# martende/findex

Measured on AMD Instinct MI355X. Metric: rank_queries_per_sec, higher is better.
Workload: dtype u64

## Files before the change

findex_amd/csrc/fmx_host.h:

```cpp
#pragma once
#include <hip/hip_runtime.h>
#include <stdint.h>

#include <atomic>
#include <memory>
#include <mutex>
#include <string>
#include <vector>

#include "fmx_device.h"
#include "fmx_hostpar.h"

namespace fmx {

struct CallCtx {
  static constexpr int kBufs = 8;
  hipStream_t stream = nullptr;
  hipEvent_t ev_a = nullptr, ev_b = nullptr;
  void *buf[kBufs] = {nullptr};
  size_t cap[kBufs] = {0};
  std::vector<hipEvent_t> chunk_ev;
  void *pin = nullptr;
  size_t pin_cap = 0;
  size_t total() const { size_t t = 0; for (size_t c : cap) t += c; return t; }
};

struct KTab {
  const uint4 *tab = nullptr;
  const uint4 *level[16] = {nullptr};
  const uint4 *const *level_dev = nullptr;
  const uint8_t *dense = nullptr;
  uint32_t k = 0, sigma = 0;
  const unsigned long long *row1 = nullptr;
  const uint4 *ext = nullptr, *ovf = nullptr;
  uint32_t ext_k = 0;
};

struct HostRank {
  std::vector<uint8_t> blob;
  size_t stride = 0;
};

struct TablePolicy {
  std::atomic<int> ktab{1};
  std::atomic<int> ktab_ext{-1};
  std::atomic<int> jump_mode{7};
  std::atomic<int> jump_pairs{-1};
  std::atomic<int> search_lanes{-1};
  std::atomic<int> jump_chars{9};
  std::atomic<long long> tables_after{-1};
  std::atomic<uint64_t> budget_bytes{~0ull};
  std::atomic<uint32_t> budget_ppb{0};
  std::atomic<int> locate_sample{32};
  TablePolicy() = default;
  TablePolicy(const TablePolicy &o) { *this = o; }
  TablePolicy &operator=(const TablePolicy &o) {
    ktab.store(o.ktab.load()); ktab_ext.store(o.ktab_ext.load()); jump_mode.store(o.jump_mode.load()); jump_pairs.store(o.jump_pairs.load());
    search_lanes.store(o.search_lanes.load());
    jump_chars.store(o.jump_chars.load()); tables_after.store(o.tables_after.load());
    budget_bytes.store(o.budget_bytes.load()); budget_ppb.store(o.budget_ppb.load());
    locate_sample.store(o.locate_sample.load());
    return *this;
  }
};
TablePolicy &default_policy();
int policy_set(TablePolicy &p, const char *key, const char *value, const char **why);

struct Index {
  uint64_t serial = 0;
  int device = 0;
  int cu_count = 256;
  uint64_t n = 0, eof = 0, nblocks = 0;
  uint32_t nslots = 0;
  int64_t counts[256] = {0};
  uint64_t cf[256] = {0};
  uint16_t slot[256] = {0};
  bool block_mode = false;
  int64_t block_bs[256] = {0};
  int block_first = -1;
  int block_skipped = -1;
  uint32_t layout = 0;
  void *d_bv = nullptr;
  void *d_chk = nullptr;
  void *d_sup = nullptr;
  void *d_bwt = nullptr;
  void *d_cf = nullptr;
  void *d_slot = nullptr;
  unsigned long long *d_counters = nullptr;
  DevIndex dev{};
  uint64_t index_bytes = 0;
  double build_ms = 0.0;
  mutable std::mutex mu;
  mutable std::vector<CallCtx *> ctx_pool;
  mutable std::mutex kt_mu;
  mutable bool kt_ready = false;
  mutable KTab kt;
  mutable void *d_ktab = nullptr, *d_kt_dense = nullptr, *d_kt_levels = nullptr;
  mutable void *d_kt_ext = nullptr, *d_kt_ovf = nullptr;
  mutable uint64_t kt_bytes = 0;
  mutable std::mutex jt_mu;
  mutable bool jt_ready = false;
  mutable void *d_jump = nullptr;
  mutable uint64_t jump_bytes = 0;
  mutable bool jump_pairs = false;
  mutable uint32_t jump_chars = 0;
  mutable std::mutex r1_mu;
  mutable bool r1_ready = false;
  mutable void *d_row1 = nullptr;
  mutable uint64_t row1_bytes = 0;
  mutable std::mutex r3_mu;
  mutable bool r3_ready = false;
  mutable void *d_row3 = nullptr;
  mutable uint64_t row3_bytes = 0;
  mutable double tables_ms = 0.0;
  mutable std::mutex tix_mu;
  mutable void *tix_owner[16] = {};
  mutable bool tix_used[16] = {};
  mutable std::atomic<uint64_t> patterns_seen{0};
  mutable std::atomic<uint32_t> search_residency{0};
  mutable std::atomic<bool> prepared_ktab{false}, prepared_rows{false};
  mutable TablePolicy policy;
  mutable std::atomic<uint64_t> tables_held{0};
  mutable std::atomic<uint64_t> tables_alloc_us{0};
  mutable std::atomic<uint64_t> hbm_free_after_tables{0};
  mutable std::atomic<uint64_t> peak_table_build_bytes{0};
  mutable std::mutex sel_mu;
  mutable bool sel_ready = false;
  mutable void *d_sel_dir = nullptr, *d_sel_off = nullptr, *d_sel_shift = nullptr;
  mutable uint64_t sel_bytes = 0;
  mutable std::mutex loc_mu;
  mutable bool loc_ready = false;
  mutable void *d_loc_marks = nullptr;
  mutable void *d_loc_samples = nullptr;
  mutable uint32_t loc_rate = 0;
  mutable bool loc_wide = false;
  mutable uint64_t loc_bytes = 0;
  mutable double loc_build_ms = 0.0;
  mutable std::mutex lcp_mu;
  mutable bool lcp_ready = false;
  mutable void *d_lcp = nullptr;
  mutable uint64_t lcp_bytes = 0;
  mutable double lcp_build_ms = 0.0;
  mutable uint32_t lcp_max = 0;
  mutable uint64_t lcp_max_row = 0, lcp_sum = 0;
  mutable uint64_t launches = 0;
  mutable double last_kernel_ms = 0.0;
  mutable std::unique_ptr<Worker> worker;
  mutable std::mutex hr_mu;
  mutable std::unique_ptr<HostRank> hr;
};

Worker *worker_of(const Index *h);

void set_error(const std::string &msg);
CallCtx *ctx_acquire(const Index *h);
void ctx_release(const Index *h, CallCtx *c);
hipError_t ctx_scratch(CallCtx *c, int i, size_t bytes, void **out);
struct CtxLease {
  const Index *h;
  CallCtx *c;
  explicit CtxLease(const Index *hh) : h(hh), c(ctx_acquire(hh)) {}
  ~CtxLease() { if (c) ctx_release(h, c); }
  CtxLease(const CtxLease &) = delete;
  CtxLease &operator=(const CtxLease &) = delete;
};
bool tables_due(const Index *h, uint64_t k, bool small_table);
void note_table_build(const Index *h, uint64_t bytes_held);
uint64_t table_room(const Index *h, uint64_t margin);
void tables_account(const Index *h, int64_t delta);
hipError_t table_malloc(const Index *h, void **p, size_t bytes);
hipError_t ktab_get(const Index *h, hipStream_t st, KTab *out, bool build = true);
hipError_t select_prepare(const Index *h, hipStream_t st);
hipError_t jump_get(const Index *h, hipStream_t st, const uint4 **out, bool build = true);
hipError_t row1_get(const Index *h, hipStream_t st, const unsigned long long **out, bool build = true);
hipError_t row3_get(const Index *h, hipStream_t st, const unsigned long long **out, bool build = true);
int drop_tables(Index *h, unsigned what);

int locate_check(const Index *h);
int locate_prepare(const Index *h, hipStream_t st);
void locate_drop(Index *h);
int locate_write_sa(const Index *h, hipStream_t st, uint32_t *d_sa_be);
uint64_t locate_write_sa_bytes(const Index *h);
hipError_t launch_locate(const Index *h, const void *d_rows, uint64_t k, void *d_out, hipStream_t st);
hipError_t launch_locate_intervals(const Index *h, const void *d_sp, const void *d_ep, uint64_t k, uint64_t max_per,
                                   void *d_off, void *d_pos, uint64_t cap, hipStream_t st);
int locate_invert_text(const Index *h, hipStream_t st, uint32_t *d_sa, uint8_t *d_s);
uint64_t locate_invert_text_bytes(const Index *h);

// ... 122 lines not shown
```

findex_amd/csrc/fmx_ktab.hip:

```cpp
#include "fmx_device.h"
#include "fmx_host.h"

#include <algorithm>
#include <chrono>
#include <cstdlib>

namespace fmx {

constexpr int kKtThreads = 256;

template <bool WIDE, uint32_t LAYOUT>
__global__ __launch_bounds__(kKtThreads) void k_ktab_level(DevIndex ix, const uint4 *__restrict__ prev, uint4 *__restrict__ next,
                                                            uint64_t n_prev, uint32_t sigma, uint32_t level,
                                                            const uint8_t *__restrict__ sym_of , uint32_t full) {
  __shared__ uint64_t s_cf[256];
  __shared__ uint16_t s_slot[256];
  for (int c = threadIdx.x; c < 256; c += blockDim.x) { s_cf[c] = ix.cf[c]; s_slot[c] = ix.slot[c]; }
  __syncthreads();
  constexpr int G = Lay<LAYOUT>::G;
  const LaneConst lc = lane_const<G>();
  const uint64_t total = n_prev * sigma;
  const uint64_t ngroups = (uint64_t)gridDim.x * (kKtThreads / G);
  for (uint64_t e = ((uint64_t)blockIdx.x * kKtThreads + threadIdx.x) / G; e < total; e += ngroups) {
    const uint64_t code = e / sigma;
    const uint32_t c = sym_of[e % sigma];
    uint64_t sp, ep;
    uint32_t steps;
    if (level == 0) { sp = 0; ep = ix.n; steps = 0; }
    else {
      const uint4 p = prev[code];
      sp = (((uint64_t)p.y << 32) | p.x) & ((1ull << 56) - 1);
      steps = p.y >> 24;
      ep = ((uint64_t)p.w << 32) | p.z;
    }
    if (sp < ep || full) {
      backward_step<WIDE, LAYOUT>(ix, c, s_slot[c], s_cf[c], lc, sp, ep);
      steps++;
    }
    if (lc.t == 0)
      next[e] = make_uint4((uint32_t)sp, (uint32_t)(sp >> 32) | (steps << 24), (uint32_t)ep, (uint32_t)(ep >> 32));
  }
}

constexpr uint32_t kExtCap = 26, kExtMaxList = 64;

template <bool WIDE, uint32_t LAYOUT>
__global__ __launch_bounds__(kKtThreads) void k_kext_head(DevIndex ix, const uint4 *__restrict__ prev, uint4 *__restrict__ ext,
                                                           uint64_t n_prev, uint32_t sigma, const uint8_t *__restrict__ sym_of,
                                                           unsigned long long *__restrict__ units) {
  __shared__ uint64_t s_cf[256];
  __shared__ uint16_t s_slot[256];
  for (int c = threadIdx.x; c < 256; c += blockDim.x) { s_cf[c] = ix.cf[c]; s_slot[c] = ix.slot[c]; }
  __syncthreads();
  constexpr int G = Lay<LAYOUT>::G;
  const LaneConst lc = lane_const<G>();
  const uint64_t total = n_prev * sigma;
  const uint64_t ngroups = (uint64_t)gridDim.x * (kKtThreads / G);
  for (uint64_t e = ((uint64_t)blockIdx.x * kKtThreads + threadIdx.x) / G; e < total; e += ngroups) {
    const uint32_t c = sym_of[e % sigma];
    uint64_t sp = 0, ep = ix.n;
    if (prev) {
      const uint4 p = prev[e / sigma];
      sp = (((uint64_t)p.y << 32) | p.x) & ((1ull << 56) - 1);
      ep = ((uint64_t)p.w << 32) | p.z;
    }
    backward_step<WIDE, LAYOUT>(ix, c, s_slot[c], s_cf[c], lc, sp, ep);
    if (lc.t == 0) {
      const uint64_t cnt = ep - sp;
      uint4 lo = make_uint4((uint32_t)sp, ((uint32_t)(sp >> 32) & 0xFFu) | ((uint32_t)cnt << 8) | 0xFFFF0000u, ~0u, ~0u);
      if (cnt > kExtCap) {
        const uint64_t off = atomicAdd(units, (unsigned long long)((cnt + 15) / 16));
        atomicMax(units + 1, (unsigned long long)cnt);
        lo = make_uint4((uint32_t)sp, ((uint32_t)(sp >> 32) & 0xFFu) | 0xFF00u | ((uint32_t)off << 16),
                        ((uint32_t)(off >> 16) & 0xFFFFFFu) | ((uint32_t)cnt << 24), (uint32_t)(cnt >> 8));
      }
      ext[2 * e] = lo;
      ext[2 * e + 1] = make_uint4(~0u, ~0u, ~0u, ~0u);
    }
  }
}

template <bool WIDE, uint32_t LAYOUT>
__global__ __launch_bounds__(kKtThreads) void k_kext_fill(DevIndex ix, const uint4 *__restrict__ ext, uint8_t *__restrict__ extb,
                                                           uint8_t *__restrict__ ovf, const uint8_t *__restrict__ dense,
                                                           uint32_t sigma, uint32_t K) {
  __shared__ uint64_t s_cf[256];
  __shared__ uint16_t s_slot[256];
  __shared__ uint8_t s_dense[256];
  for (int c = threadIdx.x; c < 256; c += blockDim.x) { s_cf[c] = ix.cf[c]; s_slot[c] = ix.slot[c]; s_dense[c] = dense[c]; }
  __syncthreads();
  constexpr int G = Lay<LAYOUT>::G;
  const LaneConst lc = lane_const<G>();
  const uint64_t ngroups = (uint64_t)gridDim.x * (kKtThreads / G);
  for (uint64_t r0 = ((uint64_t)blockIdx.x * kKtThreads + threadIdx.x) / G; r0 < ix.n; r0 += ngroups) {
    uint64_t r = r0, code = 0;
    bool ok = true;
    for (uint32_t s = 0; s < K && ok; s++) {
      const uint32_t c = r == ix.eof ? 0u : ix.bwt[r];
      const uint32_t d = s_dense[c];
      ok = d != 0xFFu;
      if (ok) {
        code = code * sigma + d;
        r = s_cf[c] + rank_excl<WIDE, LAYOUT>(ix, c, s_slot[c], r, lc);
      }
    }
    if (!ok || lc.t != 0) continue;
    uint32_t f = 0;
    for (uint32_t step = 128; step; step >>= 1)
      if (s_cf[f + step] <= r0) f += step;
    const uint4 hd = ext[2 * code];
    const uint64_t sp = hd.x | ((uint64_t)(hd.y & 0xFFu) << 32);
    const uint64_t slot = r - sp;
    if (((hd.y >> 8) & 0xFFu) != 0xFFu) {
      extb[32 * code + 6 + slot] = (uint8_t)f;
    } else {
      const uint64_t off = (hd.y >> 16) | ((uint64_t)(hd.z & 0xFFFFFFu) << 16);
      ovf[16 * off + slot] = (uint8_t)f;
    }
  }
}

static void build_kext(const Index *h, hipStream_t st, uint32_t KE, const uint8_t *d_sym, const uint8_t *d_dense) {
  const int mode = h->policy.ktab_ext.load(std::memory_order_relaxed);
  if (mode == 0 || KE == 0 || h->layout != kLayoutOneHot || h->block_mode || h->n > (1ull << 32)) return;
  const uint32_t sigma = h->nslots;
  uint64_t codes = 1;
  for (uint32_t j = 0; j < KE; j++) codes *= sigma;
  const uint64_t ext_bytes = codes * 32, ovf_reserve = std::max<uint64_t>(ext_bytes / 32, 64ull << 20);
  if (ext_bytes > (16ull << 30)) return;
  if (mode < 0) {
    const int pcfg = h->policy.jump_pairs.load(std::memory_order_relaxed);
    const bool pairs = (pcfg < 0 ? h->n >= (1ull << 30) : pcfg != 0) && (h->policy.jump_mode.load(std::memory_order_relaxed) & 6) == 6;
    if (!pairs || ext_bytes + ovf_reserve + 40 * h->n + (8ull << 30) > table_room(h, 0)) return;
  } else if (ext_bytes + ovf_reserve > table_room(h, 1ull << 30)) {
    return;
  }
  const uint64_t per_wg = kKtThreads / 4;
  auto grid_for = [&](uint64_t items) { return (int)std::min<uint64_t>((items + per_wg - 1) / per_wg, (uint64_t)h->cu_count * 8); };
  uint64_t tmp_entries = 0;
  for (uint64_t j = 1, c = sigma; j < KE; j++, c *= sigma) tmp_entries += c;
  void *d_ext = nullptr, *d_ovf = nullptr, *d_tmp = nullptr, *d_units = nullptr;
  hipError_t e = table_malloc(h, &d_ext, ext_bytes);
  if (e == hipSuccess) e = hipMalloc(&d_tmp, std::max<uint64_t>(tmp_entries, 1) * 16 + 256);
  if (e == hipSuccess) { d_units = static_cast<uint8_t *>(d_tmp) + std::max<uint64_t>(tmp_entries, 1) * 16; e = hipMemsetAsync(d_units, 0, 16, st); }
  uint64_t off = 0, n_prev = 1;
  const uint4 *prev = nullptr;
  for (uint32_t lv = 0; lv + 1 < KE && e == hipSuccess; lv++) {
    uint4 *next = static_cast<uint4 *>(d_tmp) + off;
    const uint64_t n_next = n_prev * sigma;
    const int grid = grid_for(n_next);
#define CALL(W, L) k_ktab_level<W, L><<<grid, kKtThreads, 0, st>>>(h->dev, prev, next, n_prev, sigma, lv, d_sym, 1u)
    FMX_LAYOUT_DISPATCH(h, CALL);
#undef CALL
    e = hipGetLastError();
    prev = next;
    off += n_next;
    n_prev = n_next;
  }
  if (e == hipSuccess) {
    const int grid = grid_for(codes);
#define CALL(W, L) k_kext_head<W, L><<<grid, kKtThreads, 0, st>>>(h->dev, prev, static_cast<uint4 *>(d_ext), n_prev, sigma, d_sym, static_cast<unsigned long long *>(d_units))
    FMX_LAYOUT_DISPATCH(h, CALL);
#undef CALL
    e = hipGetLastError();
  }
  unsigned long long units[2] = {0, 0};
  if (e == hipSuccess) e = hipMemcpyAsync(units, d_units, 16, hipMemcpyDeviceToHost, st);
  if (e == hipSuccess) e = hipStreamSynchronize(st);
  if (e == hipSuccess && units[1] > kExtMaxList) e = hipErrorNotSupported;
  const uint64_t ovf_bytes = std::max<uint64_t>(units[0], 1) * 16;
  if (e == hipSuccess && ovf_bytes > table_room(h, mode < 0 ? 40 * h->n + (8ull << 30) : (1ull << 30))) e = hipErrorOutOfMemory;
  if (e == hipSuccess) e = table_malloc(h, &d_ovf, ovf_bytes);
  if (e == hipSuccess) e = hipMemsetAsync(d_ovf, 0xFF, ovf_bytes, st);
  if (e == hipSuccess) {
    const int grid = grid_for(h->n);
#define CALL(W, L) k_kext_fill<W, L><<<grid, kKtThreads, 0, st>>>(h->dev, static_cast<const uint4 *>(d_ext), static_cast<uint8_t *>(d_ext), static_cast<uint8_t *>(d_ovf), d_dense, sigma, KE)
    FMX_LAYOUT_DISPATCH(h, CALL);
#undef CALL
    e = hipGetLastError();
  }
  if (e == hipSuccess) e = hipStreamSynchronize(st);
  if (d_tmp) (void)hipFree(d_tmp);
  if (e != hipSuccess) {
    (void)hipGetLastError();
    if (d_ext) (void)hipFree(d_ext);
    if (d_ovf) (void)hipFree(d_ovf);
    return;
  }
  h->d_kt_ext = d_ext;
  h->d_kt_ovf = d_ovf;
  h->kt.ext = static_cast<const uint4 *>(d_ext);
  h->kt.ovf = static_cast<const uint4 *>(d_ovf);
  h->kt.ext_k = KE;
  h->kt_bytes += ext_bytes + ovf_bytes;
  note_table_build(h, ext_bytes + ovf_bytes + tmp_entries * 16);
  tables_account(h, (int64_t)(ext_bytes + ovf_bytes));
}

static hipError_t build_ktab(const Index *h, hipStream_t st) {
  const uint32_t sigma = h->nslots;
  h->kt.k = 0;
  h->kt.sigma = sigma;
  static const int forced = getenv("FMX_KTAB") ? atoi(getenv("FMX_KTAB")) : -1;
  if (sigma < 2 || forced == 0 || !h->policy.ktab.load(std::memory_order_relaxed)) return hipSuccess;
  size_t free_b = 0, total_b = 0;
  hipError_t e = hipMemGetInfo(&free_b, &total_b);
  if (e != hipSuccess) return e;
  const uint64_t room = table_room(h, 0);
  const uint64_t share = std::max<uint64_t>(room / 4, std::min<uint64_t>(room, 64ull << 20));
  const uint64_t max_bytes = std::min<uint64_t>(std::min<uint64_t>(16ull << 30, free_b / 4), share);
  uint32_t k = 0;
  uint64_t entries = 1, all = 0;
  for (;;) {
    const uint64_t nxt = entries * sigma;
    if (k >= 16 || nxt > h->n / 8 || nxt > (1ull << 32) || (all + nxt) * 16 > max_bytes) break;
    if (forced > 0 && k >= (uint32_t)forced) break;
    entries = nxt;
    all += nxt;
    k++;
  }
  if (forced > 0)
    while (k < (uint32_t)forced && k < 16 && (all + entries * sigma) * 16 <= max_bytes) { entries *= sigma; all += entries; k++; }
  if (k == 0) return hipSuccess;
  uint8_t dense[256], sym_of[256];
  for (int c = 0; c < 256; c++) {
    dense[c] = 0xFF;
    if (h->slot[c] < kSlotEof) { dense[c] = (uint8_t)h->slot[c]; sym_of[h->slot[c]] = (uint8_t)c; }
  }
  void *d_all = nullptr, *d_dense = nullptr, *d_sym = nullptr;
  e = table_malloc(h, &d_all, all * 16);
  if (e == hipSuccess) e = hipMalloc(&d_dense, 256);
  if (e == hipSuccess) e = hipMalloc(&d_sym, 256);
  if (e == hipSuccess) e = hipMemcpyAsync(d_dense, dense, 256, hipMemcpyHostToDevice, st);
  if (e == hipSuccess) e = hipMemcpyAsync(d_sym, sym_of, 256, hipMemcpyHostToDevice, st);
  uint64_t off = 0, n_prev = 1;
  const uint4 *prev = nullptr;
  for (uint32_t lv = 0; lv < k && e == hipSuccess; lv++) {
    uint4 *next = static_cast<uint4 *>(d_all) + off;
    const uint64_t n_next = n_prev * sigma;
    const uint64_t per_wg = kKtThreads / (h->layout == kLayoutBytes ? 8 : 4);
    const int grid = (int)std::min<uint64_t>((n_next + per_wg - 1) / per_wg, (uint64_t)h->cu_count * 8);
#define CALL(W, L) k_ktab_level<W, L><<<grid, kKtThreads, 0, st>>>(h->dev, prev, next, n_prev, sigma, lv, (const uint8_t *)d_sym, 0u)
    FMX_LAYOUT_DISPATCH(h, CALL);
#undef CALL
    e = hipGetLastError();
    h->kt.level[lv] = next;
    prev = next;
    off += n_next;
    n_prev = n_next;
  }
  void *d_levels = nullptr;
  if (e == hipSuccess) e = hipMalloc(&d_levels, sizeof h->kt.level);
  if (e == hipSuccess) e = hipMemcpyAsync(d_levels, h->kt.level, sizeof h->kt.level, hipMemcpyHostToDevice, st);
  if (e == hipSuccess) e = hipStreamSynchronize(st);
  if (e != hipSuccess) {
    if (d_sym) (void)hipFree(d_sym);
    if (d_all) (void)hipFree(d_all);
    if (d_dense) (void)hipFree(d_dense);
    if (d_levels) (void)hipFree(d_levels);
    h->kt.k = 0;
    return e;
  }
  h->d_ktab = d_all;
  h->d_kt_dense = d_dense;
  h->d_kt_levels = d_levels;
  h->kt.level_dev = static_cast<const uint4 *const *>(d_levels);
  h->kt.k = k;
  h->kt.tab = h->kt.level[k - 1];
  h->kt.dense = static_cast<const uint8_t *>(d_dense);
  h->kt_bytes = all * 16 + 256;
  note_table_build(h, h->kt_bytes);
  tables_account(h, (int64_t)h->kt_bytes);
  build_kext(h, st, k >= 12 ? 12u : k >= 8 ? 8u : k >= 4 ? 4u : 0u, static_cast<const uint8_t *>(d_sym), static_cast<const uint8_t *>(d_dense));
  (void)hipFree(d_sym);
  return hipSuccess;
}

hipError_t ktab_get(const Index *h, hipStream_t st, KTab *out, bool build) {
  std::lock_guard<std::mutex> lk(h->kt_mu);
  if (!h->kt_ready && !build) {
    *out = KTab{};
    out->sigma = h->nslots;
    return hipSuccess;
  }
  if (!h->kt_ready) {
    const auto t0 = std::chrono::steady_clock::now();
    const hipError_t e = build_ktab(h, st);
    if (e != hipSuccess) {
      (void)hipGetLastError();
      h->kt = KTab{};
      h->kt.sigma = h->nslots;
    }
    h->tables_ms += std::chrono::duration<double, std::milli>(std::chrono::steady_clock::now() - t0).count();
    h->kt_ready = true;
  }
  *out = h->kt;
  return hipSuccess;
}

}
```

findex_amd/csrc/fmx_search4.h:

```cpp
#pragma once
#include <type_traits>
#include "fmx_device.h"

namespace fmx {

constexpr int kSThreads = 256;

__device__ __forceinline__ uint32_t fetch4(const uint8_t *__restrict__ pat, uint64_t pos) {
  if (pos >= 4) {
    uint32_t d;
    __builtin_memcpy(&d, pat + pos - 4, 4);
    return __builtin_bswap32(d);
  }
  uint32_t r = 0;
  for (uint32_t j = 0; j < (uint32_t)pos; j++) r |= (uint32_t)pat[pos - 1 - j] << (8 * j);
  return r;
}


__device__ __forceinline__ uint32_t pat_chunk(const uint8_t *__restrict__ pat, const uint64_t *__restrict__ own,
                                              uint64_t end, uint32_t len, uint32_t j) {
  const uint32_t have = len > 4u * j ? len - 4u * j : 0u;
  const uint64_t pos = end - 4ull * j;
  const uint32_t back = have >= 4u ? 4u : have;
// ... 428 lines not shown
      const unsigned long long wm = __builtin_amdgcn_ballot_w64(walks);
      const uint32_t slot0 = npark;
      for (uint32_t base = 0; base < take; base += P) {
        if (((wm >> base) & ((1ull << P) - 1ull)) == 0ull) continue;
        const bool actw = ((wm >> (base + grp)) & 1ull) != 0ull;
        const uint32_t gslot = slot0 + base + (actw ? grp : 0u);
        const uint64_t grow = s_park_row[wave_in_wg][gslot];
        const uint32_t gpid = s_park_pid[wave_in_wg][gslot], git = s_park_it[wave_in_wg][gslot];
        const uint32_t gnst = actw ? (uint32_t)(grow >> 56) & 15u : 0u;
        const bool gfinal = ((uint32_t)(grow >> 60) & 1u) != 0u;
        const int from = (int)(base + grp);
        const uint64_t gchars = ((uint64_t)(uint32_t)__shfl((int)(uint32_t)(chars >> 32), from, 64) << 32) | (uint32_t)__shfl((int)(uint32_t)chars, from, 64);
        uint64_t gsp = grow & ((1ull << 56) - 1);
        uint64_t gep = gsp + 1u;
        for (uint32_t s8 = 0; s8 < 8; s8++) {
          const bool stepping = actw && gsp < gep && s8 < gnst;
          if (!__builtin_amdgcn_ballot_w64(stepping)) break;
          if (stepping) walk_step((uint32_t)(gchars >> (8u * s8)) & 0xFFu, gsp, gep);
        }
        const bool again = actw && gsp < gep && !gfinal;
        if (actw && !again && t == 0) emit(gpid, gsp, gep);
        const unsigned long long am = __builtin_amdgcn_ballot_w64(again && t == 0);
        if (am) {
          const uint32_t ps = npark + (uint32_t)__builtin_popcountll(am & ((1ull << lane64) - 1ull));
          if (again && t == 0) { s_park_row[wave_in_wg][ps] = gsp; s_park_pid[wave_in_wg][ps] = gpid; s_park_it[wave_in_wg][ps] = git + gnst; }
          npark += (uint32_t)__builtin_popcountll(am);
        }
      }
    }
  };
#ifdef FMX_SEARCHLOG
  sl_t1 = __builtin_amdgcn_s_memrealtime();
#endif
  uint32_t batch = wave;
  Stage nxt_stage;
  {
    auto search_one_batch = [&](auto staged_tag, auto ahead_tag) {
    constexpr bool STAGED = decltype(staged_tag)::value;
    constexpr bool AHEAD = decltype(ahead_tag)::value;
    const uint32_t pid = batch * P + grp;
    const bool act = pid < k;
    const uint64_t *own = po.at(act ? pid : 0u);
    const uint64_t end = end0;
    const uint32_t len = act ? len0 : 0u;
    const uint64_t cur_base = cur.base;
    const uint32_t *const spat = s_pat[wave_in_wg][par];
    auto chunk = [&](uint32_t j) -> uint32_t {
      if constexpr (!STAGED) {
        return pat_chunk(pat, own, end, len, j);
      } else {
        const uint32_t have = len > 4u * j ? len - 4u * j : 0u;
        const uint32_t o = have ? (uint32_t)(end - 4ull * j - cur_base) + (kStagePad - 4u) : 0u;
        const uint32_t lo = spat[o >> 2], hi = spat[(o >> 2) + 1];
        const uint32_t r = __builtin_bswap32(__builtin_amdgcn_alignbyte(hi, lo, o & 3u));
        return have >= 4u ? r : (r & ((1u << (8u * have)) - 1u));
      }
    };
    auto chars4 = [&](uint32_t at) -> uint32_t {
      const uint32_t have = len > at ? len - at : 0u;
      if constexpr (STAGED) {
        const uint32_t o = have ? (uint32_t)(end - at - cur_base) + (kStagePad - 4u) : 0u;
        const uint32_t lo = spat[o >> 2], hi = spat[(o >> 2) + 1];
        const uint32_t r = __builtin_bswap32(__builtin_amdgcn_alignbyte(hi, lo, o & 3u));
        return have >= 4u ? r : (r & ((1u << (8u * have)) - 1u));
      } else {
        uint32_t r = 0;
        if (have >= 4u) {
          uint32_t d;
          __builtin_memcpy(&d, pat + (end - at - 4), 4);
          r = __builtin_bswap32(d);
        } else {
          for (uint32_t j = 0; j < have; j++) r |= (uint32_t)pat[end - at - 1 - j] << (8u * j);
        }
        return r;
      }
    };
    Tail tailq;
#pragma unroll
    for (uint32_t i = 0; i < NT; i++) {
      if constexpr (STAGED) tailq.c[i] = chunk(i);
      else if constexpr (kStage) tailq.c[i] = len > 4u * i ? fetch4(pat, end - 4ull * i) : 0u;
      else tailq.c[i] = act ? tail_ahead.c[i] : 0u;
    }
    uint32_t ch = tailq.c[0];
    uint32_t nx = chunk(KT ? KT / 4 + 1 : 1);
    auto issue_ahead = [&]() {
      if constexpr (AHEAD) {
        nxt_stage = stage_issue(end1, len1);
        if constexpr (!kStage) {
#pragma unroll
          for (uint32_t i = 0; i < NT; i++) tail_ahead.c[i] = len1 > 4u * i ? fetch4(pat, end1 - 4ull * i) : 0u;
        }
        load_off_raw((uint64_t)batch + 2ull * nwaves, raw2a, raw2b);
      }
    };
    if (KT == 0) { issue_ahead(); if constexpr (AHEAD) stage_park(nxt_stage, par ^ 1u); }
    uint64_t sp = 0, ep = ix.n;
    bool kx_parked = false;
    auto special = [&](uint64_t cfc, uint64_t vb, uint64_t x) { return cfc + ((vb == 1 && x > ix.eof) ? 1u : 0u); };
    if (KT == 0) {
      if (len > 0) {
        const uint32_t c = ch & 0xFFu;
        const uint4 e = s_tab[c];
        const uint4 e2 = s_tab[(c + 1) & 0xFFu];
        const uint64_t cfc = ((uint64_t)e.y << 32) | e.x;
        const uint64_t vb = ((uint64_t)e.w << 32) | e.z;
        const uint64_t nxt = c == 255u ? ix.n : (((uint64_t)e2.y << 32) | e2.x);
        sp = vb > 1 ? cfc : special(cfc, vb, 0);
        ep = vb > 1 ? nxt : special(cfc, vb, ix.n);
        steps++;
      }
      ch >>= 8;
    } else {
      uint32_t code = 0;
      bool elig = act && len >= KT;
#pragma unroll
      for (uint32_t j = 0; j < KT; j++) {
        const uint32_t d = s_dense[(tailq.c[j >> 2] >> (8u * (j & 3u))) & 0xFFu];
        elig = elig && d != 0xFFu;
        code = code * ksigma + d;
      }
      bool ex = false;
      uint32_t chk = 0;
      uint32_t zcode = 0;
      if constexpr (KX) {
        chk = chunk(KT / 4);
        bool ez = elig && len > KT;
#pragma unroll
        for (uint32_t j = 1; j <= KT; j++) {
          const uint32_t d = s_dense[((j < KT ? tailq.c[j < KT ? j >> 2 : 0u] : chk) >> (8u * (j & 3u))) & 0xFFu];
          ez = ez && d != 0xFFu;
          zcode = zcode * ksigma + d;
        }
        ex = ez;
      }
      const uint4 *ksrc = ktab + (elig ? code : 0u);
      if constexpr (KX) { if (ex) ksrc = kext + 2ull * zcode + (t & 1u); }
#ifdef FMX_SEARCHLOG
      if (!sl_look) sl_look = __builtin_amdgcn_s_memrealtime();
#endif
      const uint4 ent = *ksrc;
      issue_ahead();
      if (elig && !ex) {
        sp = (((uint64_t)ent.y << 32) | ent.x) & ((1ull << 56) - 1);
        ep = ((uint64_t)ent.w << 32) | ent.z;
        steps += ent.y >> 24;
      }
      ktl += (uint32_t)__builtin_popcountll(__builtin_amdgcn_ballot_w64(elig && t == 0));
      if constexpr (AHEAD) stage_park(nxt_stage, par ^ 1u);
      if constexpr (KX) {
        if (__builtin_amdgcn_ballot_w64(ex)) {
          const uint32_t half = t & 1u, y = tailq.c[0] & 0xFFu;
          const uint32_t h1 = gbc0(ent.y);
          const bool big = ((h1 >> 8) & 0xFFu) == 0xFFu;
          uint32_t lt = 0, le = 0;
          auto count16 = [&](const uint4 &w, uint32_t from) {
#pragma unroll
            for (uint32_t b = 0; b < 16; b++) {
              const uint32_t x = ((b < 4 ? w.x : b < 8 ? w.y : b < 12 ? w.z : w.w) >> (8u * (b & 3u))) & 0xFFu;
              lt += (b >= from && x < y) ? 1u : 0u;
              le += (b >= from && x <= y) ? 1u : 0u;
            }
          };
          if (ex && !big) count16(ent, half ? 0u : 6u);
          uint32_t cnt = (h1 >> 8) & 0xFFu;
          if (__builtin_amdgcn_ballot_w64(ex && big)) {
            const uint32_t h2 = gbc0(ent.z), h3 = gbc0(ent.w);
            const uint64_t off = (h1 >> 16) | ((uint64_t)(h2 & 0xFFFFFFu) << 16);
            const uint32_t bc = (h2 >> 24) | (h3 << 8);
            if (ex && big) cnt = bc;
            for (uint32_t i = 0;; i++) {
              const bool more = ex && big && 32u * i < bc;
              if (!__builtin_amdgcn_ballot_w64(more)) break;
              uint4 w = make_uint4(~0u, ~0u, ~0u, ~0u);
              if (more && 32u * i + 16u * half < bc) w = kovf[off + 2u * i + half];
              if (more) count16(w, 0u);
              ktl += (uint32_t)__builtin_popcountll(__builtin_amdgcn_ballot_w64(more && t == 0));
            }
          }
          lt = gbc0(lt) + gbc1(lt);
          le = y == 255u ? cnt : gbc0(le) + gbc1(le);
          const uint64_t spz = gbc0(ent.x) | ((uint64_t)(h1 & 0xFFu) << 32);
          if (ex) {
            sp = spz + lt;
            ep = spz + le;
          }
          const bool kxp = ex && sp >= ep;
          const unsigned long long pm = __builtin_amdgcn_ballot_w64(kxp && t == 0);
          if (pm) {
            const uint32_t slot = npark + (uint32_t)__builtin_popcountll(pm & ((1ull << lane64) - 1ull));
            if (kxp && t == 0) { s_park_row[wave_in_wg][slot] = sp | (0xFEull << 56); s_park_pid[wave_in_wg][slot] = pid; s_park_it[wave_in_wg][slot] = KT + 1u; }
            npark += (uint32_t)__builtin_popcountll(pm);
          }
          kx_parked = kxp;
          if (ex && !kxp) steps += KT + 1u;
        }
      }
      constexpr uint32_t kWalk = KX ? KT + 1u : KT;
      if (__builtin_amdgcn_ballot_w64(act && !(KX ? ex : elig))) {
        for (uint32_t j = 0; j < kWalk; j++) {
          const bool stepping = act && (KX ? (!ex && j >= (elig ? KT : 0u)) : !elig) && j < len && sp < ep;
          if (!__builtin_amdgcn_ballot_w64(stepping)) {
            if (KX && j < KT) continue;
            break;
          }
          if (stepping) {
            const uint32_t c = ((j < KT ? tailq.c[j < KT ? j >> 2 : 0u] : chk) >> (8u * (j & 3u))) & 0xFFu;
            const uint4 e = s_tab[c];
            if constexpr (G2) {
              const uint64_t cfc = ((uint64_t)e.y << 32) | e.x, vb = ((uint64_t)e.w << 32) | e.z;
              if (vb > 1) {
                uint32_t b1, b2, m1, m2;
                split448(sp, b1, m1);
                split448(ep, b2, m2);
                const Blk w1 = blk_load(vb, b1, b2 != b1 ? m1 : (m1 > m2 ? m1 : m2));
                Blk w2 = w1;
                if (b2 != b1) { w2 = blk_load(vb, b2, m2); reqs += RB; }
                sp = cfc + blk_rank(w1, m1);
                ep = cfc + blk_rank(w2, m2);
                reqs += RB;
              } else {
                const uint64_t r1 = cfc + ((vb == 1 && sp > ix.eof) ? 1u : 0u);
                ep = cfc + ((vb == 1 && ep > ix.eof) ? 1u : 0u);
                sp = r1;
              }
            } else {
              reqs += backward_step<WIDE, LAYOUT>(ix, c, s_slot[c], ((uint64_t)e.y << 32) | e.x, lc, sp, ep);
            }
            steps++;
          }
        }
      }
      if constexpr (KX) ch = chk >> 8;
      else ch = chunk(KT / 4);
    }
    constexpr uint32_t kIt0 = KX ? KT + 1u : (KT ? KT : 1u);
    uint32_t skip = 0;
    uint32_t cursor_it = kIt0;
    bool deferred = kx_parked;
    for (uint32_t it = kIt0;; it++) {
      bool alive = it < len && sp < ep;
      if constexpr (RW != 0u) {
        const bool hand = alive && (ep - sp) == 1 && (RW == 1u || (len - it) % RW == 0u);
        const unsigned long long hm = __builtin_amdgcn_ballot_w64(hand && t == 0);
        if (hm) {
          const uint32_t slot = nrows + (uint32_t)__builtin_popcountll(hm & ((1ull << lane64) - 1ull));
          if (hand && t == 0) {
            s_rows_row[wave_in_wg][slot] = sp; s_rows_end[wave_in_wg][slot] = end; s_rows_pid[wave_in_wg][slot] = pid;
            s_rows_it[wave_in_wg][slot] = it; s_rows_len[wave_in_wg][slot] = len;
          }
          nrows += (uint32_t)__builtin_popcountll(hm);
        }
        if (hand) {
          deferred = true;
          ep = sp;
          alive = false;
        }
      }
      if (!__builtin_amdgcn_ballot_w64(alive)) break;
      auto cursor_to = [&](uint32_t ni) {
        const uint32_t c0 = chars4(ni), a = ni & 3u;
        ch = a ? (c0 & ((1u << (8u * (4u - a))) - 1u)) : c0;
        nx = chunk((ni >> 2) + 1);
        cursor_it = ni;
      };
      auto chars12 = [&](uint32_t at, bool want, uint32_t &q0, uint32_t &q1, uint32_t &q2) {
        if constexpr (STAGED) {
          const uint32_t o = want ? (uint32_t)(end - at - cur_base) + (kStagePad - 12u) : 0u;
          const uint32_t w0 = o >> 2, sh = o & 3u;
          const uint32_t d0 = spat[w0], d1 = spat[w0 + 1], d2 = spat[w0 + 2], d3 = spat[w0 + 3];
          q0 = __builtin_bswap32(__builtin_amdgcn_alignbyte(d3, d2, sh));
          q1 = __builtin_bswap32(__builtin_amdgcn_alignbyte(d2, d1, sh));
          q2 = __builtin_bswap32(__builtin_amdgcn_alignbyte(d1, d0, sh));
        } else {
          q0 = chars4(at); q1 = chars4(at + 4u); q2 = chars4(at + 8u);
        }
      };
      const uint32_t rem = len - it;
      bool lookedup = false;
      bool park_now = false;
      uint32_t missj = 0;
      uint32_t park_ahead = 0;
      if (JT && !__builtin_amdgcn_ballot_w64(alive && (skip != 0u || (ep - sp) > (uint64_t)RG))) {
        const bool can = alive && rem >= jc;
        if (__builtin_amdgcn_ballot_w64(can)) {
          constexpr bool kPair = JT == 2u && STAGED && (G == 4 || G == 2);
          const uint64_t width = ep - sp;
          const bool single = !__builtin_amdgcn_ballot_w64(can && width != 1u);
          const uint32_t half = (kPair && single) ? (t & 1u) : 0u;
          const bool can2 = kPair && single && can && rem >= 2u * jc;
          uint32_t p0, p1, p2;
          chars12(it + (half && can2 ? jc : 0u), can, p0, p1, p2);
          const uint32_t m2 = jc > 8u ? ((1u << (8u * (jc - 8u))) - 1u) : 0u;
          bool jumped = false, pair_both = false, pair_then_miss = false;
          uint64_t rowj = 0;
          uint32_t nrows = 1;
          if (single) {
            uint4 je = make_uint4(0, 0, 0, 0);
            if (can) je = jtab[(JT == 2u ? 2ull * sp : sp) + (half && can2 ? 1u : 0u)];
            const uint32_t d0 = je.x ^ p0, d1 = je.y ^ p1, d2 = (je.z ^ p2) & m2;
            jumped = can && (d0 | d1 | d2) == 0u;
            missj = d0 ? (uint32_t)__builtin_ctz(d0) >> 3 : (d1 ? 4u + ((uint32_t)__builtin_ctz(d1) >> 3) : 8u + ((uint32_t)__builtin_ctz(d2 | 0x80000000u) >> 3));
            rowj = (uint64_t)(je.z >> 24) | ((uint64_t)je.w << 8);
            if constexpr (kPair) {
              const uint32_t ok = jumped ? 1u : 0u;
              const bool ok1 = gbc0(ok) != 0u, ok2 = can2 && gbc1(ok) != 0u;
              const uint32_t rlo1 = gbc0((uint32_t)rowj), rhi1 = gbc0((uint32_t)(rowj >> 32));
              const uint32_t rlo2 = gbc1((uint32_t)rowj), rhi2 = gbc1((uint32_t)(rowj >> 32));
              const uint32_t mj1 = gbc0(missj), mj2 = gbc1(missj);
              jumped = can && ok1;
              pair_both = ok1 && ok2;
              pair_then_miss = can2 && ok1 && !ok2;
              rowj = pair_both ? (((uint64_t)rhi2 << 32) | rlo2) : (((uint64_t)rhi1 << 32) | rlo1);
              missj = pair_then_miss ? mj2 : mj1;
            }
            jtl += (uint32_t)__builtin_popcountll(__builtin_amdgcn_ballot_w64(can && t == 0));
          } else {
            const uint32_t lane64g = threadIdx.x & 63u, gbase = lane64g - t;
            if constexpr (G2) {
              const bool mn0 = can && (uint64_t)t < width, mn1 = can && (uint64_t)(2u + t) < width;
              uint4 j0 = make_uint4(0, 0, 0, 0), j1 = make_uint4(0, 0, 0, 0);
              if (mn0) j0 = jtab[JT == 2u ? 2ull * (sp + t) : sp + t];
              if (mn1) j1 = jtab[JT == 2u ? 2ull * (sp + 2u + t) : sp + 2u + t];
              const uint32_t d0 = j0.x ^ p0, d1 = j0.y ^ p1, d2 = (j0.z ^ p2) & m2;
              const bool hit0 = mn0 && (d0 | d1 | d2) == 0u;
              const bool hit1 = mn1 && ((j1.x ^ p0) | (j1.y ^ p1) | ((j1.z ^ p2) & m2)) == 0u;
              missj = d0 ? (uint32_t)__builtin_ctz(d0) >> 3 : (d1 ? 4u + ((uint32_t)__builtin_ctz(d1) >> 3) : 8u + ((uint32_t)__builtin_ctz(d2 | 0x80000000u) >> 3));
              const uint32_t hm = ((uint32_t)(__builtin_amdgcn_ballot_w64(hit0) >> gbase) & 3u) | (((uint32_t)(__builtin_amdgcn_ballot_w64(hit1) >> gbase) & 3u) << 2);
              const uint32_t fr = hm ? (uint32_t)__builtin_ctz(hm) : 0u;
              const uint4 js = (fr >> 1) ? j1 : j0;
              const int first = (int)(gbase + (fr & 1u));
              const uint32_t rlo = (uint32_t)__shfl((int)((js.z >> 24) | (js.w << 8)), first, 64), rhi = (uint32_t)__shfl((int)(js.w >> 24), first, 64);
              jumped = can && hm != 0u;
              rowj = ((uint64_t)rhi << 32) | rlo;
// ... 358 lines not shown
```

Before: 605,000.

## Add bitmap form for extension table entries with mid-size alphabets

For alphabets with more than 26 and up to 128 symbols, extension table entries store a 128-bit presence bitmap of distinct following symbols plus up to ten repeat bytes, rather than every occurrence symbol. Entries that overflow are demoted to the overflow list through a spill buffer and a two-pass demote kernel. At search time, lt/le counts come from popcounts over the bitmap and the repeats using SWAR byte compares. This is meant to keep more codes inside the 32-byte entry and avoid overflow reads, at the cost of a more complex build with atomics and extra device syncs.

```diff
diff --git a/findex_amd/csrc/fmx_host.h b/findex_amd/csrc/fmx_host.h
--- a/findex_amd/csrc/fmx_host.h
+++ b/findex_amd/csrc/fmx_host.h
@@ -33,7 +33,7 @@
   uint32_t k = 0, sigma = 0;
   const unsigned long long *row1 = nullptr;
   const uint4 *ext = nullptr, *ovf = nullptr;
-  uint32_t ext_k = 0;
+  uint32_t ext_k = 0, ext_form = 0;
 };
 
 struct HostRank {
diff --git a/findex_amd/csrc/fmx_ktab.hip b/findex_amd/csrc/fmx_ktab.hip
--- a/findex_amd/csrc/fmx_ktab.hip
+++ b/findex_amd/csrc/fmx_ktab.hip
@@ -43,11 +43,15 @@
 }
 
 constexpr uint32_t kExtCap = 26, kExtMaxList = 64;
+constexpr uint32_t kExtRepeats = 10;
+constexpr uint64_t kExtSpillCap = 1ull << 20;
+
+static uint32_t kext_bitmap_form(uint32_t sigma) { return sigma > kExtCap && sigma <= 128u ? 1u : 0u; }
 
 template <bool WIDE, uint32_t LAYOUT>
 __global__ __launch_bounds__(kKtThreads) void k_kext_head(DevIndex ix, const uint4 *__restrict__ prev, uint4 *__restrict__ ext,
                                                            uint64_t n_prev, uint32_t sigma, const uint8_t *__restrict__ sym_of,
-                                                           unsigned long long *__restrict__ units) {
+                                                           unsigned long long *__restrict__ units, uint32_t form) {
   __shared__ uint64_t s_cf[256];
   __shared__ uint16_t s_slot[256];
   for (int c = threadIdx.x; c < 256; c += blockDim.x) { s_cf[c] = ix.cf[c]; s_slot[c] = ix.slot[c]; }
@@ -68,6 +72,12 @@
     if (lc.t == 0) {
       const uint64_t cnt = ep - sp;
       uint4 lo = make_uint4((uint32_t)sp, ((uint32_t)(sp >> 32) & 0xFFu) | ((uint32_t)cnt << 8) | 0xFFFF0000u, ~0u, ~0u);
+      if (form) {
+        if (cnt > kExtCap) atomicMax(units + 1, (unsigned long long)cnt);
+        ext[2 * e] = make_uint4((uint32_t)sp, ((uint32_t)(sp >> 32) & 0xFFu) | 0x8000u | 0xFFFF0000u, ~0u, ~0u);
+        ext[2 * e + 1] = make_uint4(0u, 0u, 0u, 0u);
+        continue;
+      }
       if (cnt > kExtCap) {
         const uint64_t off = atomicAdd(units, (unsigned long long)((cnt + 15) / 16));
         atomicMax(units + 1, (unsigned long long)cnt);
@@ -83,7 +93,8 @@
 template <bool WIDE, uint32_t LAYOUT>
 __global__ __launch_bounds__(kKtThreads) void k_kext_fill(DevIndex ix, const uint4 *__restrict__ ext, uint8_t *__restrict__ extb,
                                                            uint8_t *__restrict__ ovf, const uint8_t *__restrict__ dense,
-                                                           uint32_t sigma, uint32_t K) {
+                                                           uint32_t sigma, uint32_t K, uint32_t form,
+                                                           unsigned long long *__restrict__ spill, unsigned long long *__restrict__ units) {
   __shared__ uint64_t s_cf[256];
   __shared__ uint16_t s_slot[256];
   __shared__ uint8_t s_dense[256];
@@ -108,6 +119,23 @@
     uint32_t f = 0;
     for (uint32_t step = 128; step; step >>= 1)
       if (s_cf[f + step] <= r0) f += step;
+    if (form) {
+      uint32_t *w = reinterpret_cast<uint32_t *>(extb + 32 * code);
+      const uint32_t d = s_dense[f];
+      if (d == 0xFFu) { atomicOr(w + 1, 0x4000u); continue; }
+      const uint32_t bit = 1u << (d & 31u);
+      if (!(atomicOr(w + 4 + (d >> 5), bit) & bit)) continue;
+      const uint32_t idx = (atomicAdd(w + 1, 0x100u) >> 8) & 0x3Fu;
+      if (idx < kExtRepeats) {
+        const uint32_t b = 6u + idx;
+        atomicAnd(w + (b >> 2), ~(0xFFu << (8u * (b & 3u))) | (d << (8u * (b & 3u))));
+      } else {
+        if (idx == kExtRepeats) atomicAdd(units + 3, 1ull);
+        const unsigned long long at = atomicAdd(units + 2, 1ull);
+        if (at < kExtSpillCap) spill[at] = code | ((unsigned long long)d << 32) | ((unsigned long long)idx << 40);
+      }
+      continue;
+    }
     const uint4 hd = ext[2 * code];
     const uint64_t sp = hd.x | ((uint64_t)(hd.y & 0xFFu) << 32);
     const uint64_t slot = r - sp;
@@ -116,6 +144,38 @@
     } else {
       const uint64_t off = (hd.y >> 16) | ((uint64_t)(hd.z & 0xFFFFFFu) << 16);
       ovf[16 * off + slot] = (uint8_t)f;
+    }
+  }
+}
+
+__global__ __launch_bounds__(kKtThreads) void k_kext_demote(uint32_t *__restrict__ ext, uint8_t *__restrict__ ovf,
+                                                             const unsigned long long *__restrict__ spill, uint64_t nspill,
+                                                             const uint8_t *__restrict__ sym_of, unsigned long long *__restrict__ units,
+                                                             uint32_t pass) {
+  for (uint64_t i = (uint64_t)blockIdx.x * kKtThreads + threadIdx.x; i < nspill; i += (uint64_t)gridDim.x * kKtThreads) {
+    const unsigned long long rec = spill[i];
+    uint32_t *w = ext + 8ull * (rec & 0xFFFFFFFFull);
+    const uint32_t d = (uint32_t)(rec >> 32) & 0xFFu, idx = (uint32_t)(rec >> 40);
+    if (pass == 0) {
+      if (idx != kExtRepeats) continue;
+      const uint32_t mk = (w[1] >> 8) & 0xFFu;
+      const uint64_t off = atomicAdd(units, (unsigned long long)(kExtMaxList / 16));
+      uint8_t *o = ovf + 16 * off;
+      uint32_t pos = 0;
+      for (uint32_t j = 0; j < 4; j++)
+        for (uint32_t m = w[4 + j]; m; m &= m - 1) o[pos++] = sym_of[32u * j + (uint32_t)__builtin_ctz(m)];
+      for (uint32_t b = 6; b < 16; b++) o[pos++] = sym_of[(w[b >> 2] >> (8u * (b & 3u))) & 0xFFu];
+      if (mk & 0x40u) o[pos++] = 0;
+      o[pos++] = sym_of[d];
+      const uint32_t cnt = pos + (mk & 0x3Fu) - (kExtRepeats + 1u);
+      w[1] = (w[1] & 0xFFu) | 0xFF00u | ((uint32_t)off << 16);
+      w[2] = ((uint32_t)(off >> 16) & 0xFFFFFFu) | (cnt << 24);
+      w[3] = cnt >> 8;
+      w[4] = pos;
+      w[5] = w[6] = w[7] = ~0u;
+    } else if (idx != kExtRepeats) {
+      const uint64_t off = (w[1] >> 16) | ((uint64_t)(w[2] & 0xFFFFFFu) << 16);
+      ovf[16 * off + atomicAdd(w + 4, 1u)] = sym_of[d];
     }
   }
 }
@@ -157,30 +217,58 @@
     off += n_next;
     n_prev = n_next;
   }
-  if (e == hipSuccess) {
-    const int grid = grid_for(codes);
-#define CALL(W, L) k_kext_head<W, L><<<grid, kKtThreads, 0, st>>>(h->dev, prev, static_cast<uint4 *>(d_ext), n_prev, sigma, d_sym, static_cast<unsigned long long *>(d_units))
-    FMX_LAYOUT_DISPATCH(h, CALL);
-#undef CALL
-    e = hipGetLastError();
-  }
-  unsigned long long units[2] = {0, 0};
-  if (e == hipSuccess) e = hipMemcpyAsync(units, d_units, 16, hipMemcpyDeviceToHost, st);
-  if (e == hipSuccess) e = hipStreamSynchronize(st);
-  if (e == hipSuccess && units[1] > kExtMaxList) e = hipErrorNotSupported;
-  const uint64_t ovf_bytes = std::max<uint64_t>(units[0], 1) * 16;
+  uint32_t form = kext_bitmap_form(sigma);
+  unsigned long long units[4] = {0, 0, 0, 0};
+  void *d_spill = nullptr;
+  for (;; form = 0) {
+    if (e == hipSuccess) e = hipMemsetAsync(d_units, 0, sizeof units, st);
+    if (e == hipSuccess) {
+      const int grid = grid_for(codes);
+#define CALL(W, L) k_kext_head<W, L><<<grid, kKtThreads, 0, st>>>(h->dev, prev, static_cast<uint4 *>(d_ext), n_prev, sigma, d_sym, static_cast<unsigned long long *>(d_units), form)
+      FMX_LAYOUT_DISPATCH(h, CALL);
+#undef CALL
+      e = hipGetLastError();
+    }
+    if (e == hipSuccess) e = hipMemcpyAsync(units, d_units, sizeof units, hipMemcpyDeviceToHost, st);
+    if (e == hipSuccess) e = hipStreamSynchronize(st);
+    if (e == hipSuccess && units[1] > kExtMaxList) e = hipErrorNotSupported;
+    if (!form || e != hipSuccess) break;
+    e = hipMalloc(&d_spill, kExtSpillCap * 8);
+    if (e == hipSuccess) {
+      const int grid = grid_for(h->n);
+#define CALL(W, L) k_kext_fill<W, L><<<grid, kKtThreads, 0, st>>>(h->dev, static_cast<const uint4 *>(d_ext), static_cast<uint8_t *>(d_ext), nullptr, d_dense, sigma, KE, 1u, static_cast<unsigned long long *>(d_spill), static_cast<unsigned long long *>(d_units))
+      FMX_LAYOUT_DISPATCH(h, CALL);
+#undef CALL
+      e = hipGetLastError();
+    }
+    if (e == hipSuccess) e = hipMemcpyAsync(units, d_units, sizeof units, hipMemcpyDeviceToHost, st);
+    if (e == hipSuccess) e = hipStreamSynchronize(st);
+    if (e != hipSuccess || units[2] <= kExtSpillCap) break;
+    (void)hipFree(d_spill);
+    d_spill = nullptr;
+  }
+  const uint64_t ovf_bytes = form ? std::max<uint64_t>(units[3], 1) * kExtMaxList : std::max<uint64_t>(units[0], 1) * 16;
   if (e == hipSuccess && ovf_bytes > table_room(h, mode < 0 ? 40 * h->n + (8ull << 30) : (1ull << 30))) e = hipErrorOutOfMemory;
   if (e == hipSuccess) e = table_malloc(h, &d_ovf, ovf_bytes);
   if (e == hipSuccess) e = hipMemsetAsync(d_ovf, 0xFF, ovf_bytes, st);
-  if (e == hipSuccess) {
+  if (e == hipSuccess && form && units[2]) {
+    const int grid = (int)std::min<uint64_t>((units[2] + kKtThreads - 1) / kKtThreads, (uint64_t)h->cu_count * 8);
+    for (uint32_t pass = 0; pass < 2 && e == hipSuccess; pass++) {
+      k_kext_demote<<<grid, kKtThreads, 0, st>>>(static_cast<uint32_t *>(d_ext), static_cast<uint8_t *>(d_ovf), static_cast<const unsigned long long *>(d_spill),
+                                                 units[2], d_sym, static_cast<unsigned long long *>(d_units), pass);
+      e = hipGetLastError();
+    }
+  }
+  if (e == hipSuccess && !form) {
     const int grid = grid_for(h->n);
-#define CALL(W, L) k_kext_fill<W, L><<<grid, kKtThreads, 0, st>>>(h->dev, static_cast<const uint4 *>(d_ext), static_cast<uint8_t *>(d_ext), static_cast<uint8_t *>(d_ovf), d_dense, sigma, KE)
+#define CALL(W, L) k_kext_fill<W, L><<<grid, kKtThreads, 0, st>>>(h->dev, static_cast<const uint4 *>(d_ext), static_cast<uint8_t *>(d_ext), static_cast<uint8_t *>(d_ovf), d_dense, sigma, KE, 0u, nullptr, nullptr)
     FMX_LAYOUT_DISPATCH(h, CALL);
 #undef CALL
     e = hipGetLastError();
   }
   if (e == hipSuccess) e = hipStreamSynchronize(st);
   if (d_tmp) (void)hipFree(d_tmp);
+  if (d_spill) (void)hipFree(d_spill);
   if (e != hipSuccess) {
     (void)hipGetLastError();
     if (d_ext) (void)hipFree(d_ext);
@@ -192,6 +280,7 @@
   h->kt.ext = static_cast<const uint4 *>(d_ext);
   h->kt.ovf = static_cast<const uint4 *>(d_ovf);
   h->kt.ext_k = KE;
+  h->kt.ext_form = form;
   h->kt_bytes += ext_bytes + ovf_bytes;
   note_table_build(h, ext_bytes + ovf_bytes + tmp_entries * 16);
   tables_account(h, (int64_t)(ext_bytes + ovf_bytes));
diff --git a/findex_amd/csrc/fmx_search4.h b/findex_amd/csrc/fmx_search4.h
--- a/findex_amd/csrc/fmx_search4.h
+++ b/findex_amd/csrc/fmx_search4.h
@@ -604,7 +604,9 @@
         if (__builtin_amdgcn_ballot_w64(ex)) {
           const uint32_t half = t & 1u, y = tailq.c[0] & 0xFFu;
           const uint32_t h1 = gbc0(ent.y);
-          const bool big = ((h1 >> 8) & 0xFFu) == 0xFFu;
+          const uint32_t mk = (h1 >> 8) & 0xFFu;
+          const bool big = mk == 0xFFu;
+          const bool bits = ex && !big && (mk & 0x80u) != 0u;
           uint32_t lt = 0, le = 0;
           auto count16 = [&](const uint4 &w, uint32_t from) {
 #pragma unroll
@@ -614,7 +616,29 @@
               le += (b >= from && x <= y) ? 1u : 0u;
             }
           };
-          if (ex && !big) count16(ent, half ? 0u : 6u);
+          if (__builtin_amdgcn_ballot_w64(ex && !big && !bits)) {
+            if (ex && !big && !bits) count16(ent, half ? 0u : 6u);
+          }
+          if (__builtin_amdgcn_ballot_w64(bits)) {
+            const uint32_t yd = s_dense[y];
+            uint32_t l, e;
+            if (half) {
+              auto below = [&](uint32_t w, uint32_t i) {
+                const int s = (int)yd - (int)(32u * i);
+                return (uint32_t)__builtin_popcount(w & (s <= 0 ? 0u : s >= 32 ? ~0u : (1u << s) - 1u));
+              };
+              l = below(ent.x, 0) + below(ent.y, 1) + below(ent.z, 2) + below(ent.w, 3);
+              const uint32_t wy = yd < 64u ? (yd < 32u ? ent.x : ent.y) : (yd < 96u ? ent.z : ent.w);
+              e = l + ((wy >> (yd & 31u)) & 1u);
+            } else {
+              const uint32_t v0 = yd * 0x01010101u, v1 = v0 + 0x01010101u, hi = 0x80808080u;
+              const uint32_t a = ent.y | 0xFFFFu, b = ent.z, c = ent.w;
+              const uint32_t eof = (mk >> 6) & 1u;
+              l = eof + (uint32_t)(__builtin_popcount(~((a | hi) - v0) & hi) + __builtin_popcount(~((b | hi) - v0) & hi) + __builtin_popcount(~((c | hi) - v0) & hi));
+              e = eof + (uint32_t)(__builtin_popcount(~((a | hi) - v1) & ~a & hi) + __builtin_popcount(~((b | hi) - v1) & ~b & hi) + __builtin_popcount(~((c | hi) - v1) & ~c & hi));
+            }
+            if (bits) { lt = l; le = e; }
+          }
           uint32_t cnt = (h1 >> 8) & 0xFFu;
           if (__builtin_amdgcn_ballot_w64(ex && big)) {
             const uint32_t h2 = gbc0(ent.z), h3 = gbc0(ent.w);
@@ -631,7 +655,7 @@
             }
           }
           lt = gbc0(lt) + gbc1(lt);
-          le = y == 255u ? cnt : gbc0(le) + gbc1(le);
+          le = (y == 255u && !bits) ? cnt : gbc0(le) + gbc1(le);
           const uint64_t spz = gbc0(ent.x) | ((uint64_t)(h1 & 0xFFu) << 32);
           if (ex) {
             sp = spz + lt;
```

Result: slower. 596,800 (-1.4%).
